# zqqqqz2000/MixGRPO

Hardware: AMD Instinct MI355X
Metric: GRPO train-step images/sec, FLUX.1-dev 1024^2 (higher is better)
Workload: dtype bf16

## Files before the change

### mixgrpo_amd/csrc/gemm.hip

```cpp
#include "../../include/mixgrpo_hip.h"
#include "common.h"

#include <cmath>
#include <cstdlib>

namespace {

constexpr int BM = 128, BN = 128, BK = 64;
constexpr int NT = 256;

struct RowMap {
  long ld;
  long rpb;
  long bstride;
};

__device__ __forceinline__ long row_off(const RowMap& r, long m) {
  const uint32_t rpb = (uint32_t)r.rpb;
  const uint32_t b = (uint32_t)m / rpb;
  return (long)b * r.bstride + (long)((uint32_t)m - b * rpb) * r.ld;
}

enum Epi { EPI_BIAS = 0, EPI_BIAS_GELU = 1, EPI_BIAS_GATE_RES = 2, EPI_F32_ACC = 3, EPI_BIAS_MULAUX = 4,
           EPI_QKNORM = 5 ,
// ... 458 lines not shown
  for (int j = 0; j < AHEAD; ++j) load_cs(j, j, dep0);
  __builtin_amdgcn_sched_barrier(0);
  float ssq[MT];
#pragma unroll
  for (int j = 0; j < MT; ++j) {
    float x[16], p[8];
    unpack8(y[j][0], x);
    unpack8(y[j][1], x + 8);
#pragma unroll
    for (int i = 0; i < 8; ++i)
      p[i] = PAIRED ? vadd1(vmul1(x[2 * i], x[2 * i]), vmul1(x[2 * i + 1], x[2 * i + 1])) : x[2 * i] * x[2 * i] + x[2 * i + 1] * x[2 * i + 1];
    float sacc = PAIRED ? vadd1(vadd1(vadd1(p[0], p[1]), vadd1(p[2], p[3])), vadd1(vadd1(p[4], p[5]), vadd1(p[6], p[7])))
                        : ((p[0] + p[1]) + (p[2] + p[3])) + ((p[4] + p[5]) + (p[6] + p[7]));
    sacc += __shfl_xor(sacc, 16, 64);
    sacc += __shfl_xor(sacc, 32, 64);
    ssq[j] = sacc;
    if (j & 1) __builtin_amdgcn_sched_barrier(0);
  }
  {
    float* wr = reinterpret_cast<float*>(red + (wu ^ 1) * 1024);
    const float* rd = reinterpret_cast<const float*>(red + wu * 1024);
    if (fq == 0) {
#pragma unroll
      for (int j = 0; j < MT; ++j) wr[fr + 16 * j] = ssq[j];
    }
    __builtin_amdgcn_sched_barrier(0);
    asm volatile("s_waitcnt lgkmcnt(0)" ::: "memory");
    __builtin_amdgcn_s_barrier();
    __builtin_amdgcn_sched_barrier(0);
#pragma unroll
    for (int j = 0; j < MT; ++j) ssq[j] = ssq[j] + rd[fr + 16 * j];
  }
  bf16_raw* out = (sec ? g.qn_K : g.qn_Q) + (((long)bu * g.qn_H + head) * g.qn_S + g.qn_s0 + t0 + fr) * 128 + hb;
#pragma unroll
  for (int j = 0; j < MT; ++j) {
    const int slot = j % NSLOT;
    if (j + AHEAD < MT) {
      uint32_t dep = 0;
      if (j > 0) asm volatile("" : "+v"(dep) : "v"(y[j - 1][1].w));
      load_cs((j + AHEAD) % NSLOT, j + AHEAD, dep);
    }
    __builtin_amdgcn_sched_barrier(0);
    const float r = rsqrtf(ssq[j] / 128.f + 1e-6f);
    float x[16], o[16];
    unpack8(y[j][0], x);
    unpack8(y[j][1], x + 8);
    if constexpr (PAIRED) {
#pragma unroll
      for (int q4 = 0; q4 < 4; ++q4) {
        const float4 v = cs[slot][q4];
#pragma unroll
        for (int h = 0; h < 2; ++h) {
          const int i = 2 * q4 + h;
          const float cv = h ? v.z : v.x, sv = h ? v.w : v.y;
          const float y0 = vmul1(vmul1(x[2 * i], r), wv[2 * i]), y1 = vmul1(vmul1(x[2 * i + 1], r), wv[2 * i + 1]);
          o[2 * i] = vsub1(vmul1(y0, cv), vmul1(y1, sv));
          o[2 * i + 1] = vadd1(vmul1(y1, cv), vmul1(y0, sv));
        }
      }
    } else {
#pragma unroll
      for (int q4 = 0; q4 < 4; ++q4) {
        const float4 cv = cs[slot][q4], sv = cs[slot][4 + q4];
        const float c[4] = {cv.x, cv.y, cv.z, cv.w}, sn[4] = {sv.x, sv.y, sv.z, sv.w};
#pragma unroll
        for (int h = 0; h < 2; ++h) {
          const int i = 2 * q4 + h;
          const float y0 = x[2 * i] * r * wv[2 * i], y1 = x[2 * i + 1] * r * wv[2 * i + 1];
          o[2 * i] = y0 * c[2 * h] - y1 * sn[2 * h];
          o[2 * i + 1] = y1 * c[2 * h + 1] + y0 * sn[2 * h + 1];
        }
      }
    }
    y[j][0] = pack8(o);
    y[j][1] = pack8(o + 8);
    if (inside) {
      *reinterpret_cast<uint4*>(out + (long)j * 16 * 128 + f0) = y[j][0];
      *reinterpret_cast<uint4*>(out + (long)j * 16 * 128 + f1) = y[j][1];
    }
    __builtin_amdgcn_sched_barrier(0);
  }
}

template <int EPI>
__device__ __forceinline__ void persist_epilogue(const GemmArgs& g, f32x4 (&acc)[4][8], int wid, int lane, long m0,
                                                 long n0, char* red = nullptr) {
  if constexpr (EPI == EPI_QKNORM || EPI == EPI_QKNORM_P) {
    qknorm_epilogue<EPI == EPI_QKNORM_P>(g, acc, wid, lane, m0, n0, red);
    return;
  }
  constexpr int MT = 8;
  const int wm = wid >> 2, wn = wid & 3, fr = lane & 15, fq = lane >> 4;
  const long nw = n0 + wn * 64;
  const long mrow0 = m0 + wm * 128 + fr;

  if (EPI == EPI_F32_ACC) {
    float* Cb = reinterpret_cast<float*>(g.C);
    const bool rmw = g.beta != 0.f;
    bool nok[4];
    long ncol[4];
#pragma unroll
    for (int t = 0; t < 4; ++t) {
      nok[t] = nw + lane_feat(fq, t) < g.N;
      ncol[t] = nok[t] ? nw + lane_feat(fq, t) : 0;
    }
#pragma unroll
    for (int jb = 0; jb < MT; jb += 2) {
      long off[2];
      bool rok[2];
      float4 old[2][4];
#pragma unroll
      for (int jj = 0; jj < 2; ++jj) {
        const long m = mrow0 + (jb + jj) * 16;
        rok[jj] = m < g.M;
        off[jj] = rok[jj] ? row_off(g.c, m) : 0;
      }
      if (rmw) {
#pragma unroll
        for (int jj = 0; jj < 2; ++jj)
#pragma unroll
          for (int t = 0; t < 4; ++t) old[jj][t] = *reinterpret_cast<const float4*>(Cb + off[jj] + ncol[t]);
      }
#pragma unroll
      for (int jj = 0; jj < 2; ++jj)
#pragma unroll
        for (int t = 0; t < 4; ++t) {
          const f32x4 a = acc[t][jb + jj];
          float4 o = make_float4(a[0], a[1], a[2], a[3]);
          if (rmw) {
            o.x = vfma1(g.beta, old[jj][t].x, o.x);
            o.y = vfma1(g.beta, old[jj][t].y, o.y);
            o.z = vfma1(g.beta, old[jj][t].z, o.z);
            o.w = vfma1(g.beta, old[jj][t].w, o.w);
          }
          if (rok[jj] && nok[t]) *reinterpret_cast<float4*>(Cb + off[jj] + ncol[t]) = o;
        }
    }
    return;
  }

  if (!g.rowwise_ok) {
#pragma unroll
    for (int j = 0; j < MT; ++j) {
      const long m = mrow0 + j * 16;
      if (m >= g.M) continue;
      const long crow = row_off(g.c, m);
      const long bidx = (uint32_t)m / (uint32_t)g.c.rpb;
#pragma unroll
      for (int t = 0; t < 4; ++t) {
        const long nn = nw + lane_feat(fq, t);
        if (nn >= g.N) continue;
        float v[4] = {acc[t][j][0], acc[t][j][1], acc[t][j][2], acc[t][j][3]};
        if (g.bias) {
          const uint2 bb = *reinterpret_cast<const uint2*>(g.bias + nn);
          v[0] += bf2f(bb.x & 0xffff); v[1] += bf2f(bb.x >> 16); v[2] += bf2f(bb.y & 0xffff); v[3] += bf2f(bb.y >> 16);
        }
#pragma unroll
        for (int r = 0; r < 4; ++r) v[r] = rbf(v[r]);
        bf16_raw* cp = reinterpret_cast<bf16_raw*>(g.C) + crow + nn;
        uint2 pre;
        pre.x = (uint32_t)f2bf(v[0]) | ((uint32_t)f2bf(v[1]) << 16);
        pre.y = (uint32_t)f2bf(v[2]) | ((uint32_t)f2bf(v[3]) << 16);
        if (EPI == EPI_BIAS_GELU) {
          if (g.aux) *reinterpret_cast<uint2*>(g.aux + m * g.ldaux + nn) = pre;
#pragma unroll
          for (int r = 0; r < 4; ++r) v[r] = gelu_tanh_f(v[r]);
        } else if (EPI == EPI_BIAS_GATE_RES) {
          if (g.aux) *reinterpret_cast<uint2*>(g.aux + m * g.ldaux + nn) = pre;
          const uint2 gg = *reinterpret_cast<const uint2*>(g.gate + bidx * g.gate_ld + nn);
// ... 63 lines not shown
    }
  };
  if (SIDE) {
    load_side(0, 0, 0);
    load_side(1, 2, 0);
  }
  __builtin_amdgcn_sched_barrier(0);
  uint4 y[MT][2];
  {
    float bias[16];
    unpack8(bias0, bias);
    unpack8(bias1, bias + 8);
    if (brows) {
#pragma unroll
      for (int j = 0; j < MT; ++j) {
        float v[16];
#pragma unroll
        for (int t = 0; t < 4; ++t)
#pragma unroll
          for (int r = 0; r < 4; ++r) v[t * 4 + r] = acc[t][j][r] + brow[j];
        y[j][0] = pack8(v);
        y[j][1] = pack8(v + 8);
        __builtin_amdgcn_sched_barrier(0);
      }
    } else {
#pragma unroll
      for (int j = 0; j < MT; ++j) {
        float v[16];
#pragma unroll
        for (int t = 0; t < 4; ++t)
#pragma unroll
          for (int r = 0; r < 4; ++r) v[t * 4 + r] = acc[t][j][r] + bias[t * 4 + r];
        y[j][0] = pack8(v);
        y[j][1] = pack8(v + 8);
        __builtin_amdgcn_sched_barrier(0);
      }
    }
  }
#pragma unroll
  for (int jb = 0; jb < MT; jb += 2) {
    const int slot = (jb >> 1) & 1;
    uint4 o[2][2];
#pragma unroll
    for (int jj = 0; jj < 2; ++jj) {
      const int j = jb + jj;
      if (EPI == EPI_BIAS) {
        o[jj][0] = y[j][0];
        o[jj][1] = y[j][1];
      } else {
        float v[16];
        unpack8(y[j][0], v);
        unpack8(y[j][1], v + 8);
        if (EPI == EPI_BIAS_GELU) {
#pragma unroll
          for (int e = 0; e < 16; ++e) v[e] = gelu_tanh_f(v[e]);
        } else if (EPI == EPI_BIAS_GATE_RES) {
          float gv[16], rv[16];
          unpack8(gate0, gv);
          unpack8(gate1, gv + 8);
          unpack8(side[slot][SIDE ? jj : 0][0], rv);
          unpack8(side[slot][SIDE ? jj : 0][1], rv + 8);
#pragma unroll
          for (int e = 0; e < 16; ++e) v[e] = rv[e] + rbf(gv[e] * v[e]);
        } else if (EPI == EPI_BIAS_MULAUX) {
          float pv[16];
          unpack8(side[slot][SIDE ? jj : 0][0], pv);
          unpack8(side[slot][SIDE ? jj : 0][1], pv + 8);
#pragma unroll
          for (int e = 0; e < 16; ++e) v[e] *= gelu_tanh_grad_f(pv[e]);
        }
        o[jj][0] = pack8(v);
        o[jj][1] = pack8(v + 8);
      }
    }
    if (SIDE && jb + 4 < MT) {
      uint32_t dep = 0;
      asm volatile("" : "+v"(dep) : "v"(o[1][1].w));
      load_side(slot, jb + 4, dep);
    }
#pragma unroll
    for (int jj = 0; jj < 2; ++jj) {
      const int j = jb + jj;
      const int r = fr + 16 * j;
      if (r <= rmax) {
        char* cb = const_cast<char*>(cbase);
        const uint32_t co = (uint32_t)r * ldc2;
        if ((EPI == EPI_BIAS_GELU || EPI == EPI_BIAS_GATE_RES) && g.aux) {
          char* ab = const_cast<char*>(abase);
          const uint32_t ao = (uint32_t)r * lda2;
          if (nok0) *reinterpret_cast<uint4*>(ab + (ao + c0)) = y[j][0];
          if (nok1) *reinterpret_cast<uint4*>(ab + (ao + c1)) = y[j][1];
        }
        if (nok0) *reinterpret_cast<uint4*>(cb + (co + c0)) = o[jj][0];
        if (nok1) *reinterpret_cast<uint4*>(cb + (co + c1)) = o[jj][1];
      }
    }
    __builtin_amdgcn_sched_barrier(0);
  }
}


constexpr int SK_PMAX = 8;
constexpr long SK_SLOT = 256L * 256;

__host__ __device__ inline int sk_parts(int R, int nw) { return R > 0 ? (nw / R < SK_PMAX ? nw / R : SK_PMAX) : 0; }
__host__ __device__ inline bool sk_on(const float* ws, int minparts, int R, int nw, int nkt) {
  const int P = sk_parts(R, nw);
  return ws != nullptr && P >= 2 && P >= minparts && nkt >= 4 * P;
}

struct SkTail {
  int nfull;
  int nseg;
  int tile0, k00, k01, part0;
  int tile1, k11;
};

__device__ __forceinline__ SkTail sk_tail(const GemmArgs& g, int xcnt, int nw, int w, int nkt) {
  SkTail t;
  t.nfull = xcnt / nw;
  const int R = xcnt - t.nfull * nw, base = t.nfull * nw;
  t.nseg = 0; t.tile0 = 0; t.k00 = 0; t.k01 = nkt; t.part0 = 0; t.tile1 = 0; t.k11 = nkt;
  if (!sk_on(g.sk_ws, g.sk_minparts, R, nw, nkt)) {
    if (w < R) { t.nseg = 1; t.tile0 = base + w; }
    return t;
  }
  const int P = sk_parts(R, nw);
  if (w >= P * R) return t;
  const int p = w / R, r = w - p * R;
  t.nseg = 1; t.tile0 = base + r;
  t.k00 = p * nkt / P; t.k01 = (p + 1) * nkt / P;
  t.part0 = 1;
  return t;
}

template <int EPI, bool PAIR>
__global__ void __launch_bounds__(64) gemm_sk_fixup_kernel(GemmArgs g, int nw) {
  const int lane = threadIdx.x, wid = blockIdx.x & 7, xcd = (blockIdx.x >> 3) & 7, r = blockIdx.x >> 6;
  const int tiles_m = (g.M + 255) / 256, tiles_n = (g.N + 255) / 256, nwg = tiles_m * tiles_n, nkt = g.K / BK;
  const int q = nwg >> 3, rem = nwg & 7;
  const int xbeg = xcd < rem ? xcd * (q + 1) : rem * (q + 1) + (xcd - rem) * q;
  const int xcnt = xcd < rem ? q + 1 : q;
  const int nfull = xcnt / nw, R = xcnt - nfull * nw;
  if (r >= R || !sk_on(g.sk_ws, g.sk_minparts, R, nw, nkt)) return;
  const int P = sk_parts(R, nw);
  f32x4 acc[4][8];
#pragma unroll
  for (int i = 0; i < 4; ++i)
#pragma unroll
    for (int j = 0; j < 8; ++j) acc[i][j] = f32x4{0.f, 0.f, 0.f, 0.f};
  for (int p = 0; p < P; ++p) {
    const int w = p * R + r;
    const float* wsp = g.sk_ws + ((long)(w * 8 + xcd) << 16) + ((wid * 32) * 64 + lane) * 4;
#pragma unroll
    for (int i = 0; i < 4; ++i)
#pragma unroll
      for (int j = 0; j < 8; ++j) {
        const f32x4 v = *reinterpret_cast<const f32x4*>(wsp + (i * 8 + j) * 256);
        acc[i][j] += v;
      }
  }
  const int tl = xbeg + nfull * nw + r, band = g.band;
  const int per_band = band * tiles_n, b0 = tl / per_band, rows_in_band = min(band, tiles_m - b0 * band);
  const int in_band = tl - b0 * per_band;
  long m0 = (long)(b0 * band + in_band % rows_in_band) * 256;
  const long n0 = (long)(in_band / rows_in_band) * 256;
  const GemmArgs gl = seg_args<PAIR>(g, m0);
  if constexpr (EPI != EPI_QKNORM && EPI != EPI_QKNORM_P) persist_epilogue<EPI>(gl, acc, wid, lane, m0, n0);
}

template <int EPI, bool CONV, int MODE>
__global__ void __launch_bounds__(512, 2) gemm_pp_kernel(GemmArgs g) {
  constexpr bool SK = (MODE & 1) != 0, PAIR = (MODE & 2) != 0;
  constexpr int TM = 256, TN = 256, NTHR = 512, RS = NTHR / 8, TB = TM * 128, MT = 8, NTL = 4;
  constexpr int WBASE = 3 * TB;
  extern __shared__ __attribute__((aligned(16))) char smem[];
  const int tid = threadIdx.x, lane = tid & 63, wid = tid >> 6;
  const int wm = wid >> 2, wn = wid & 3;
  const int fr = lane & 15, fq = lane >> 4;
  const int tiles_m = (g.M + TM - 1) / TM, tiles_n = (g.N + TN - 1) / TN;
  const int nwg = tiles_m * tiles_n;
  const int nkt = g.K / BK;
  const int band = g.band;
  const int xcd = blockIdx.x & 7, lane_in_xcd = blockIdx.x >> 3, per_xcd_wg = gridDim.x >> 3;
  const int q = nwg >> 3, rem = nwg & 7;
  const int xbeg = xcd < rem ? xcd * (q + 1) : rem * (q + 1) + (xcd - rem) * q;
  const int xcnt = xcd < rem ? q + 1 : q;
  SkTail sk;
  if (SK) {
    sk = sk_tail(g, xcnt, per_xcd_wg, lane_in_xcd, nkt);
  } else {
    sk.nfull = lane_in_xcd < xcnt ? (xcnt - lane_in_xcd + per_xcd_wg - 1) / per_xcd_wg : 0;
    sk.nseg = 0; sk.tile0 = 0; sk.k00 = 0; sk.k01 = nkt; sk.part0 = 0; sk.tile1 = 0; sk.k11 = nkt;
  }
  const int nunits = sk.nfull + sk.nseg;
  if (nunits == 0) return;
  const int wu = __builtin_amdgcn_readfirstlane(wid);
  const bool late = wu >= 4;
  const int lrow = tid >> 3, lkc = tid & 7;
  const int src_kc = swz(lrow, lkc);
  const int wrow = wperm(lrow);
  typedef __attribute__((address_space(3))) char lds_char;
  typedef const __attribute__((address_space(1))) char gbl_char;
  uint32_t ao[4], wo[4];
  long m0, n0;
#define TILE_COORDS(tl, M0, N0)                                            \
  do {                                                                     \
    const int per_band = band * tiles_n;                                   \
    const int b0 = (tl) / per_band;                                        \
    const int rows_in_band = min(band, tiles_m - b0 * band);               \
    const int in_band = (tl) - b0 * per_band;                              \
    M0 = (long)(b0 * band + in_band % rows_in_band) * TM;                  \
    N0 = (long)(in_band / rows_in_band) * TN;                              \
  } while (0)
#define TILE_OFFS(M0, N0, AO, WO)                                                          \
  do {                                                                                     \
    _Pragma("unroll") for (int k_ = 0; k_ < 4; ++k_) {                                     \
      long mm = M0 + lrow + k_ * RS;                                                       \
      if (mm >= g.M) mm = g.M - 1;                                                         \
      const bool s2_ = PAIR && g.m_split && M0 >= g.m_split;                               \
      const long ar_ = !PAIR ? row_off(g.a, mm)                                            \
                             : (s2_ ? row_off(g.a2, mm - g.m_split) + g.a2_off : row_off(g.a, mm) + g.a1_off); \
      AO[k_] = (uint32_t)((ar_ + src_kc * 8) * 2);                                         \
      long nn = N0 + k_ * 64 + wrow;                                                       \
      if (nn >= g.N) nn = g.N - 1;                                                         \
      WO[k_] = (uint32_t)((nn * g.ldw + (!PAIR ? 0 : (s2_ ? g.w2_off : g.w1_off)) + src_kc * 8) * 2); \
    }                                                                                      \
  } while (0)
#define PGLDS(base, off, off_lds) \
  __builtin_amdgcn_global_load_lds((gbl_char*)((base) + (off)), (lds_char*)(smem + (off_lds)), 16, 0, 0)
#define PIN() __builtin_amdgcn_sched_barrier(0)
#define BAR() do { PIN(); __builtin_amdgcn_s_barrier(); PIN(); } while (0)

  uint32_t a_ro[2], w_ro[2];
#pragma unroll
  for (int ks = 0; ks < 2; ++ks) {
    a_ro[ks] = (uint32_t)((wm * 128 + fr) * 128 + (swz(fr, ks * 4 + fq) << 4));
    w_ro[ks] = (uint32_t)(WBASE + (wn * 64 + fr) * 128 + (swz(fr, ks * 4 + fq) << 4));
  }
#define LDA(ks, j) (*reinterpret_cast<const s16x8*>(smem + sa_ + a_ro[ks] + (j) * 2048))
#define LDW(ks, i) (*reinterpret_cast<const s16x8*>(smem + sw_ + w_ro[ks] + (i) * 2048))
#define MMA(i_, j_, W_, A_) acc[i_][j_] = __builtin_amdgcn_mfma_f32_16x16x32_bf16(W_, A_, acc[i_][j_], 0, 0, 0)

#define PGLDS_K PGLDS
#define LDA_K LDA
#define LDW_K LDW
#define UNIT(i, T_, K0_, K1_, P_)                                                        \
  do {                                                                                     \
    const int s_ = SK ? (i) - sk.nfull : -1;                                               \
    T_ = s_ < 0 ? lane_in_xcd + (i) * per_xcd_wg : (s_ == 0 ? sk.tile0 : sk.tile1);       \
    K0_ = s_ < 0 ? 0 : (s_ == 0 ? sk.k00 : 0);                                             \
    K1_ = s_ < 0 ? nkt : (s_ == 0 ? sk.k01 : sk.k11);                                      \
    P_ = s_ < 0 ? 0 : (s_ == 0 ? sk.part0 : 1);                                            \
  } while (0)
  int ui = 0, u_tile, kbeg, kend, partial;
  UNIT(0, u_tile, kbeg, kend, partial);
  TILE_COORDS(xbeg + u_tile, m0, n0);
  TILE_OFFS(m0, n0, ao, wo);
  {
    const char* ab = reinterpret_cast<const char*>(g.A);
    const char* wb = reinterpret_cast<const char*>(g.W) + (long)kbeg * (BK * 2);
    const int la = wu * 1024, lw = WBASE + wu * 1024;
#pragma unroll
    for (int k = 0; k < 4; ++k) PGLDS(ab + a_koff<CONV>(g, kbeg) * 2, ao[k], la + k * RS * 128);
#pragma unroll
    for (int k = 0; k < 4; ++k) PGLDS(wb, wo[k], lw + k * RS * 128);
#pragma unroll
    for (int k = 0; k < 4; ++k) PGLDS(ab + a_koff<CONV>(g, kbeg + 1) * 2, ao[k], TB + la + k * RS * 128);
#pragma unroll
    for (int k = 0; k < 4; ++k) PGLDS(wb + BK * 2, wo[k], TB + lw + k * RS * 128);
  }
  asm volatile("s_waitcnt vmcnt(0)" ::: "memory");
  __syncthreads();
  if (late) __builtin_amdgcn_s_barrier();
  int aslot = 0, wslot = 0;
  while (true) {
    const bool has_next = ui + 1 < nunits;
    long nm0 = 0, nn0 = 0;
    int n_tile = u_tile, nkbeg = kbeg, nkend = kend, npartial = partial;
    uint32_t nao[4] = {ao[0], ao[1], ao[2], ao[3]}, nwo[4] = {wo[0], wo[1], wo[2], wo[3]};
    if (has_next) {
      UNIT(ui + 1, n_tile, nkbeg, nkend, npartial);
      TILE_COORDS(xbeg + n_tile, nm0, nn0);
      TILE_OFFS(nm0, nn0, nao, nwo);
    }
    uint32_t ca[4] = {ao[0], ao[1], ao[2], ao[3]}, cw[4] = {wo[0], wo[1], wo[2], wo[3]};
    f32x4 acc[NTL][MT];
#pragma unroll
    for (int i = 0; i < NTL; ++i)
#pragma unroll
      for (int j = 0; j < MT; ++j) acc[i][j] = f32x4{0.f, 0.f, 0.f, 0.f};
    const int klen = kend - kbeg;
    for (int kt = 0; kt < klen; ++kt) {
      const bool nxt = kt + 2 >= klen;
      const int k2 = nxt ? nkbeg + (kt + 2 - klen) : kbeg + kt + 2;
#pragma unroll
      for (int k = 0; k < 4; ++k) {
        ca[k] = nxt ? nao[k] : ca[k];
        cw[k] = nxt ? nwo[k] : cw[k];
      }
      const int a_dst = aslot == 0 ? 2 : aslot - 1;
      const char* ab_ = reinterpret_cast<const char*>(g.A) + a_koff<CONV>(g, k2) * 2;
      const char* wb_ = reinterpret_cast<const char*>(g.W) + (long)k2 * (BK * 2);
      const int la_ = a_dst * TB + wu * 1024, lw_ = WBASE + wslot * TB + wu * 1024;
      const uint32_t sa_ = aslot * TB, sw_ = wslot * TB;
      s16x8 faA[2][4], faB[2][4], fw[2][4];
#pragma unroll
      for (int ks = 0; ks < 2; ++ks)
#pragma unroll
        for (int i = 0; i < 4; ++i) fw[ks][i] = LDW_K(ks, i);
#pragma unroll
      for (int ks = 0; ks < 2; ++ks)
#pragma unroll
        for (int j = 0; j < 4; ++j) faA[ks][j] = LDA_K(ks, j);
#pragma unroll
      for (int k = 0; k < 4; ++k) PGLDS_K(ab_, ca[k], la_ + k * RS * 128);
      BAR();
      __builtin_amdgcn_s_setprio(1);
#pragma unroll
      for (int ks = 0; ks < 2; ++ks)
#pragma unroll
        for (int j = 0; j < 4; ++j)
#pragma unroll
          for (int i = 0; i < 4; ++i) MMA(i, j, fw[ks][i], faA[ks][j]);
      __builtin_amdgcn_s_setprio(0);
      BAR();
#pragma unroll
      for (int ks = 0; ks < 2; ++ks)
#pragma unroll
        for (int j = 0; j < 4; ++j) faB[ks][j] = LDA_K(ks, 4 + j);
#pragma unroll
      for (int k = 0; k < 4; ++k) PGLDS_K(wb_, cw[k], lw_ + k * RS * 128);
      PIN();
      asm volatile("s_waitcnt vmcnt(8)" ::: "memory");
      BAR();
      __builtin_amdgcn_s_setprio(1);
#pragma unroll
      for (int ks = 0; ks < 2; ++ks)
#pragma unroll
        for (int j = 0; j < 4; ++j)
#pragma unroll
          for (int i = 0; i < 4; ++i) MMA(i, 4 + j, fw[ks][i], faB[ks][j]);
      __builtin_amdgcn_s_setprio(0);
      BAR();
      aslot = aslot == 2 ? 0 : aslot + 1;
      wslot ^= 1;
    }
    int el = lane, ew = wid;
    asm volatile("" : "+v"(el), "+v"(ew));
    if (SK && partial) {
      float* wsp = g.sk_ws + ((long)blockIdx.x << 16) + ((ew * 32) * 64 + el) * 4;
#pragma unroll
      for (int i = 0; i < NTL; ++i)
#pragma unroll
        for (int j = 0; j < MT; ++j) *reinterpret_cast<f32x4*>(wsp + (i * MT + j) * 256) = acc[i][j];
    } else if (PAIR) {
      long m0l = m0;
      const GemmArgs gl = seg_args<true>(g, m0l);
      persist_epilogue<EPI>(gl, acc, ew, el, m0l, n0);
    } else {
      persist_epilogue<EPI>(g, acc, ew, el, m0, n0, smem + (aslot == 0 ? 2 : aslot - 1) * TB);
    }
    if (!has_next) break;
    ++ui;
    u_tile = n_tile; kbeg = nkbeg; kend = nkend; partial = npartial;
    m0 = nm0; n0 = nn0;
#pragma unroll
    for (int k = 0; k < 4; ++k) { ao[k] = nao[k]; wo[k] = nwo[k]; }
  }
  if (!late) __builtin_amdgcn_s_barrier();
#undef UNIT
#undef TILE_COORDS
#undef TILE_OFFS
#undef PGLDS
#undef PIN
#undef BAR
#undef PGLDS_K
#undef LDA_K
#undef LDW_K
#undef LDA
#undef LDW
#undef MMA
}

bool persistent_ok(const GemmArgs& g) {
  const long tiles_big = (long)cdiv(g.M, 256) * cdiv(g.N, 256);
  static const long min_tiles = getenv("MGX_GEMM_BIG_MIN_TILES") ? atol(getenv("MGX_GEMM_BIG_MIN_TILES")) : 128;
  static const int mode = getenv("MGX_GEMM_MODE") ? atoi(getenv("MGX_GEMM_MODE")) : 9;
  const bool big = g.M >= 256 && g.N >= 256 && tiles_big >= min_tiles && (g.N % 256 == 0 || g.N >= 2048);
  return big && mode != 0 && g.span32 && g.K >= 2 * BK;
}

template <int EPI, bool CONV = false>
int launch(const GemmArgs& g_in, hipStream_t st) {
  GemmArgs g = g_in;
  {
    const int tiles_m = cdiv(g.M, 256), tiles_n = cdiv(g.N, 256);
    static const int band_env = getenv("MGX_GEMM_BAND") ? atoi(getenv("MGX_GEMM_BAND")) : 0;
    g.band = band_env > 0 ? min(band_env, tiles_m) : (g.band > 0 ? min(g.band, tiles_m) : (tiles_n <= 16 ? 1 : (tiles_m <= 16 ? tiles_m : 4)));
  }
  const long tiles_big = (long)cdiv(g.M, 256) * cdiv(g.N, 256);
  static bool attr_set = false;
  if (!attr_set) {
    (void)hipFuncSetAttribute((const void*)gemm_kernel<EPI, CONV>, hipFuncAttributeMaxDynamicSharedMemorySize, 65536);
    (void)hipFuncSetAttribute((const void*)gemm_pp_kernel<EPI, CONV, 0>, hipFuncAttributeMaxDynamicSharedMemorySize, 163840);
    if (!CONV) {
      (void)hipFuncSetAttribute((const void*)gemm_pp_kernel<EPI, false, 1>, hipFuncAttributeMaxDynamicSharedMemorySize, 163840);
      (void)hipFuncSetAttribute((const void*)gemm_pp_kernel<EPI, false, 2>, hipFuncAttributeMaxDynamicSharedMemorySize, 163840);
      (void)hipFuncSetAttribute((const void*)gemm_pp_kernel<EPI, false, 3>, hipFuncAttributeMaxDynamicSharedMemorySize, 163840);
    }
    attr_set = true;
  }
  const bool pair = !CONV && g.m_split != 0;
  if (EPI == EPI_QKNORM || EPI == EPI_QKNORM_P) g.sk_ws = nullptr;
  if (persistent_ok(g)) {
    int grid = 256;
    static const float sk_cost_us = getenv("MGX_GEMM_SK_COST_US") ? (float)atof(getenv("MGX_GEMM_SK_COST_US")) : 40.f;
    static const float sk_slow = getenv("MGX_GEMM_SK_SLOWDOWN") ? (float)atof(getenv("MGX_GEMM_SK_SLOWDOWN")) : 1.25f;
    static const int sk_off = getenv("MGX_GEMM_SK") ? atoi(getenv("MGX_GEMM_SK")) == 0 : 0;
    int rmax = 0;
    g.sk_minparts = 0;
    if (g.sk_ws && !sk_off && !CONV) {
      const float tile_us = (float)g.K * 0.0247f;
      const float room = 1.f - sk_cost_us / tile_us;
      g.sk_minparts = room <= 0.f ? SK_PMAX + 1 : (int)floorf(sk_slow / room) + 1;
      if (g.sk_minparts < 2) g.sk_minparts = 2;
      const int nw = grid / 8, q = (int)(tiles_big >> 3), rem = (int)(tiles_big & 7);
      for (int x = 0; x < 8; ++x) {
        const int cnt = x < rem ? q + 1 : q, R = cnt % nw;
        if (sk_on(g.sk_ws, g.sk_minparts, R, nw, g.K / BK) && R > rmax) rmax = R;
      }
    }
    if (rmax == 0) {
      g.sk_ws = nullptr;
      if (tiles_big < grid) grid = (int)((tiles_big + 7) / 8 * 8);
    }
    if (rmax > 0 && pair) {
      gemm_pp_kernel<EPI, false, 3><<<grid, 512, 163840, st>>>(g);
      gemm_sk_fixup_kernel<EPI, true><<<rmax * 64, 64, 0, st>>>(g, grid / 8);
    } else if (rmax > 0) {
      gemm_pp_kernel<EPI, false, 1><<<grid, 512, 163840, st>>>(g);
      gemm_sk_fixup_kernel<EPI, false><<<rmax * 64, 64, 0, st>>>(g, grid / 8);
    } else if (pair) {
      gemm_pp_kernel<EPI, false, 2><<<grid, 512, 163840, st>>>(g);
    } else {
      gemm_pp_kernel<EPI, CONV, 0><<<grid, 512, 163840, st>>>(g);
    }
  } else {
    if (pair) return 1;
    gemm_kernel<EPI, CONV><<<cdiv(g.M, BM) * cdiv(g.N, BN), NT, 65536, st>>>(g);
  }
  MGX_CHECK_LAUNCH();
  return MGX_OK;
}

__global__ void __launch_bounds__(256) gelu_rows_kernel(const bf16_raw* __restrict__ x, long ldx, bf16_raw* __restrict__ y,
                                                        long ldy, long M, int N8) {
  const long total = M * N8;
  for (long id = (long)blockIdx.x * 256 + threadIdx.x; id < total; id += (long)gridDim.x * 256) {
    const long m = id / N8;
    const int c = (int)(id - m * N8);
    const uint4 u = *reinterpret_cast<const uint4*>(x + m * ldx + c * 8);
    float v[8];
    unpack8(u, v);
#pragma unroll
    for (int e = 0; e < 8; ++e) v[e] = gelu_tanh_f(v[e]);
    *reinterpret_cast<uint4*>(y + m * ldy + c * 8) = pack8(v);
  }
}

}

extern "C" long mgx_gemm_sk_workspace_elems(void) { return 256L * SK_SLOT; }

namespace {
int dispatch(const GemmArgs& g, int epilogue, hipStream_t st) {
  switch (epilogue) {
    case EPI_BIAS: return launch<EPI_BIAS>(g, st);
    case EPI_BIAS_GELU: return launch<EPI_BIAS_GELU>(g, st);
    case EPI_BIAS_GATE_RES: return launch<EPI_BIAS_GATE_RES>(g, st);
    case EPI_F32_ACC: return launch<EPI_F32_ACC>(g, st);
    case EPI_BIAS_MULAUX: return launch<EPI_BIAS_MULAUX>(g, st);
  }
  mgx_set_error("unknown GEMM epilogue");
  return MGX_ERR_ARG;
}

bool side_ok16(int N, int M, const void* C, long ldc, long c_rpb, long c_bstride, const void* aux, long ldaux, const void* gate,
               long gate_ld, const void* bias) {
  return (N % 8 == 0) && (c_rpb >= M || c_rpb % 128 == 0) && (ldc % 8 == 0) && (c_bstride % 8 == 0) && ((uintptr_t)C % 16 == 0) &&
         (!aux || (ldaux % 8 == 0 && (uintptr_t)aux % 16 == 0)) && (!gate || (gate_ld % 8 == 0 && (uintptr_t)gate % 16 == 0)) &&
         (!bias || (uintptr_t)bias % 16 == 0);
}
}

extern "C" int mgx_gemm_bf16_sk(const uint16_t* A, const uint16_t* W, const uint16_t* bias, void* C, const uint16_t* gate,
                                uint16_t* aux, long ldaux, int M, int N, int K, long lda, long a_rpb, long a_bstride, long ldw, long ldc,
                                long c_rpb, long c_bstride, long gate_ld, int epilogue, float beta, float* sk_workspace,
                                long sk_workspace_elems, void* stream) {
  MGX_REQUIRE(A && W && C, "null operand");
  MGX_REQUIRE(!sk_workspace || (sk_workspace_elems >= mgx_gemm_sk_workspace_elems() && (uintptr_t)sk_workspace % 16 == 0),
              "stream-K workspace too small (mgx_gemm_sk_workspace_elems) or misaligned");
  MGX_REQUIRE(M > 0 && N > 0 && K > 0, "empty GEMM");
  MGX_REQUIRE(K % BK == 0, "K must be a multiple of 64");
  MGX_REQUIRE(N % 4 == 0, "N must be a multiple of 4");
  MGX_REQUIRE(lda % 8 == 0 && ldw % 8 == 0 && ldc % 4 == 0, "leading dimensions must keep 16-byte row alignment");
  MGX_REQUIRE(a_rpb > 0 && c_rpb > 0, "rows-per-batch must be positive");
  MGX_REQUIRE(!aux || ldaux % 4 == 0, "aux leading dimension must keep 8-byte alignment");
  MGX_REQUIRE(a_bstride % 8 == 0 && c_bstride % 4 == 0, "batch strides must keep alignment");
  MGX_REQUIRE(((uintptr_t)A % 16 == 0) && ((uintptr_t)W % 16 == 0) && ((uintptr_t)C % 8 == 0), "operands must be 16-byte aligned");
  MGX_REQUIRE(epilogue != EPI_BIAS_GATE_RES || gate, "gate-residual epilogue needs a gate");
  MGX_REQUIRE(epilogue != EPI_BIAS_MULAUX || aux, "gelu-backward epilogue needs the saved pre-activation");
  GemmArgs g{};
  g.A = A; g.W = W; g.bias = bias; g.C = C; g.gate = gate; g.aux = aux; g.ldaux = ldaux; g.gate_ld = gate_ld;
  g.M = M; g.N = N; g.K = K;
  const long RPB_MAX = 1L << 30;
  g.a = RowMap{lda, a_rpb < RPB_MAX ? a_rpb : RPB_MAX, a_bstride};
  g.c = RowMap{ldc, c_rpb < RPB_MAX ? c_rpb : RPB_MAX, c_bstride};
  g.ldw = ldw;
  g.beta = beta;
// ... 201 lines not shown
```

Baseline: 0.4341.

## Defer persistent GEMM epilogue stores into next tile's K-loop

In the persistent GEMM, the bf16 epilogue output of a full interior tile is kept in registers instead of being written right away. The global stores are then issued in batches during the first peeled K-iterations of the next tile, so the store traffic overlaps with MFMA work. The first MMA zeroes the accumulator in place of a separate clear, and the vmcnt waits are adjusted to cover the pending stores. The cost is more register pressure (16 uint4 per lane) and tight hand-tuned waitcnt schedules. It is enabled by default for the BIAS and BIAS_GATE_RES epilogues.

```diff
diff --git a/mixgrpo_amd/csrc/gemm.hip b/mixgrpo_amd/csrc/gemm.hip
--- a/mixgrpo_amd/csrc/gemm.hip
+++ b/mixgrpo_amd/csrc/gemm.hip
@@ -564,9 +564,15 @@
   }
 }
 
-template <int EPI>
+struct PendAddr {
+  char* cb;
+  uint32_t ldc2;
+  uint32_t off0;
+};
+template <int EPI, bool DEFER = false>
 __device__ __forceinline__ void persist_epilogue(const GemmArgs& g, f32x4 (&acc)[4][8], int wid, int lane, long m0,
-                                                 long n0, char* red = nullptr) {
+                                                 long n0, char* red = nullptr, uint4 (*pend)[2] = nullptr,
+                                                 PendAddr* pa = nullptr) {
   if constexpr (EPI == EPI_QKNORM || EPI == EPI_QKNORM_P) {
     qknorm_epilogue<EPI == EPI_QKNORM_P>(g, acc, wid, lane, m0, n0, red);
     return;
@@ -796,20 +802,30 @@
     for (int jj = 0; jj < 2; ++jj) {
       const int j = jb + jj;
       const int r = fr + 16 * j;
-      if (r <= rmax) {
+      if (DEFER || r <= rmax) {
         char* cb = const_cast<char*>(cbase);
         const uint32_t co = (uint32_t)r * ldc2;
         if ((EPI == EPI_BIAS_GELU || EPI == EPI_BIAS_GATE_RES) && g.aux) {
           char* ab = const_cast<char*>(abase);
           const uint32_t ao = (uint32_t)r * lda2;
-          if (nok0) *reinterpret_cast<uint4*>(ab + (ao + c0)) = y[j][0];
-          if (nok1) *reinterpret_cast<uint4*>(ab + (ao + c1)) = y[j][1];
+          if (DEFER || nok0) *reinterpret_cast<uint4*>(ab + (ao + c0)) = y[j][0];
+          if (DEFER || nok1) *reinterpret_cast<uint4*>(ab + (ao + c1)) = y[j][1];
         }
-        if (nok0) *reinterpret_cast<uint4*>(cb + (co + c0)) = o[jj][0];
-        if (nok1) *reinterpret_cast<uint4*>(cb + (co + c1)) = o[jj][1];
+        if constexpr (DEFER) {
+          pend[j][0] = o[jj][0];
+          pend[j][1] = o[jj][1];
+        } else {
+          if (nok0) *reinterpret_cast<uint4*>(cb + (co + c0)) = o[jj][0];
+          if (nok1) *reinterpret_cast<uint4*>(cb + (co + c1)) = o[jj][1];
+        }
       }
     }
     __builtin_amdgcn_sched_barrier(0);
+  }
+  if constexpr (DEFER) {
+    pa->cb = const_cast<char*>(cbase);
+    pa->ldc2 = (uint32_t)__builtin_amdgcn_readfirstlane((int)ldc2);
+    pa->off0 = (uint32_t)fr * ldc2 + c0;
   }
 }
 
@@ -883,9 +899,32 @@
   if constexpr (EPI != EPI_QKNORM && EPI != EPI_QKNORM_P) persist_epilogue<EPI>(gl, acc, wid, lane, m0, n0);
 }
 
-template <int EPI, bool CONV, int MODE>
+constexpr int defer_s(int epi, int i) {
+#ifdef MGX_DEFER_SCHED
+  constexpr int s[4] = MGX_DEFER_SCHED;
+  return s[i];
+#else
+  constexpr int wide[4] = {2, 1, 1, 0}, tight[4] = {2, 2, 0, 0};
+  return epi == EPI_BIAS_GATE_RES ? wide[i] : tight[i];
+#endif
+}
+constexpr int DEFER_BST = 4;
+constexpr int DEFER_AUX = 16;
+constexpr int DEFER_MINK = 4;
+constexpr bool defer_epi(int epi) { return epi == EPI_BIAS || epi == EPI_BIAS_GELU || epi == EPI_BIAS_GATE_RES || epi == EPI_BIAS_MULAUX; }
+
+template <int EPI, bool CONV, int MODE, bool DEFER = false>
 __global__ void __launch_bounds__(512, 2) gemm_pp_kernel(GemmArgs g) {
   constexpr bool SK = (MODE & 1) != 0, PAIR = (MODE & 2) != 0;
+  static_assert(!DEFER || (defer_epi(EPI) && !CONV), "only the four bf16 epilogues of the plain GEMM defer their stores");
+  constexpr int DEFER_S[4] = {defer_s(EPI, 0), defer_s(EPI, 1), defer_s(EPI, 2), defer_s(EPI, 3)};
+  constexpr int DEFER_W0 = 8 + DEFER_BST * (DEFER_S[0] + DEFER_S[1]);
+  constexpr int DEFER_W1 = 8 + DEFER_BST * (DEFER_S[1] + DEFER_S[2] + DEFER_S[3]);
+  constexpr int DEFER_W2 = 8 + DEFER_BST * DEFER_S[3];
+  constexpr int DEFER_PEEL = DEFER_S[3] > 0 ? 3 : 2;
+  static_assert(DEFER_S[0] + DEFER_S[1] + DEFER_S[2] + DEFER_S[3] == 4, "a wave's block is four 2-row batches");
+  static_assert(DEFER_W0 + DEFER_AUX <= 63 && DEFER_W1 <= 63 && DEFER_W2 <= 63, "vmcnt is a 6-bit counter");
+  static_assert(DEFER_PEEL + 1 <= DEFER_MINK, "the peeled K-iterations must exist");
   constexpr int TM = 256, TN = 256, NTHR = 512, RS = NTHR / 8, TB = TM * 128, MT = 8, NTL = 4;
   constexpr int WBASE = 3 * TB;
   extern __shared__ __attribute__((aligned(16))) char smem[];
@@ -954,7 +993,27 @@
   }
 #define LDA(ks, j) (*reinterpret_cast<const s16x8*>(smem + sa_ + a_ro[ks] + (j) * 2048))
 #define LDW(ks, i) (*reinterpret_cast<const s16x8*>(smem + sw_ + w_ro[ks] + (i) * 2048))
-#define MMA(i_, j_, W_, A_) acc[i_][j_] = __builtin_amdgcn_mfma_f32_16x16x32_bf16(W_, A_, acc[i_][j_], 0, 0, 0)
+#define MMA(i_, j_, W_, A_, Z_) \
+  acc[i_][j_] = __builtin_amdgcn_mfma_f32_16x16x32_bf16(W_, A_, (Z_) ? f32x4{0.f, 0.f, 0.f, 0.f} : acc[i_][j_], 0, 0, 0)
+  constexpr bool EPI_HAS_AUX = EPI == EPI_BIAS_GELU || EPI == EPI_BIAS_GATE_RES;
+  uint4 pend[8][2];
+  PendAddr pa;
+  bool carry = false, p_aux = false;
+#define PEND_CLEAR()                                                                                    \
+  do {                                                                                                  \
+    _Pragma("unroll") for (int j_ = 0; j_ < 8; ++j_) pend[j_][0] = pend[j_][1] = make_uint4(0, 0, 0, 0); \
+  } while (0)
+  PEND_CLEAR();
+  pa.cb = nullptr; pa.ldc2 = 0; pa.off0 = 0;
+#define PEND_STORE(b_)                                                                                  \
+  do {                                                                                                  \
+    _Pragma("unroll") for (int jj_ = 0; jj_ < 2; ++jj_) {                                               \
+      const int j_ = 2 * (b_) + jj_;                                                                    \
+      const uint32_t co_ = pa.off0 + (uint32_t)(16 * j_) * pa.ldc2;                                     \
+      *reinterpret_cast<uint4*>(pa.cb + co_) = pend[j_][0];                                             \
+      *reinterpret_cast<uint4*>(pa.cb + (co_ + 64)) = pend[j_][1];                                      \
+    }                                                                                                   \
+  } while (0)
 
 #define PGLDS_K PGLDS
 #define LDA_K LDA
@@ -1000,68 +1059,96 @@
     }
     uint32_t ca[4] = {ao[0], ao[1], ao[2], ao[3]}, cw[4] = {wo[0], wo[1], wo[2], wo[3]};
     f32x4 acc[NTL][MT];
-#pragma unroll
-    for (int i = 0; i < NTL; ++i)
-#pragma unroll
-      for (int j = 0; j < MT; ++j) acc[i][j] = f32x4{0.f, 0.f, 0.f, 0.f};
     const int klen = kend - kbeg;
-    for (int kt = 0; kt < klen; ++kt) {
-      const bool nxt = kt + 2 >= klen;
-      const int k2 = nxt ? nkbeg + (kt + 2 - klen) : kbeg + kt + 2;
-#pragma unroll
-      for (int k = 0; k < 4; ++k) {
-        ca[k] = nxt ? nao[k] : ca[k];
-        cw[k] = nxt ? nwo[k] : cw[k];
-      }
-      const int a_dst = aslot == 0 ? 2 : aslot - 1;
-      const char* ab_ = reinterpret_cast<const char*>(g.A) + a_koff<CONV>(g, k2) * 2;
-      const char* wb_ = reinterpret_cast<const char*>(g.W) + (long)k2 * (BK * 2);
-      const int la_ = a_dst * TB + wu * 1024, lw_ = WBASE + wslot * TB + wu * 1024;
-      const uint32_t sa_ = aslot * TB, sw_ = wslot * TB;
-      s16x8 faA[2][4], faB[2][4], fw[2][4];
-#pragma unroll
-      for (int ks = 0; ks < 2; ++ks)
-#pragma unroll
-        for (int i = 0; i < 4; ++i) fw[ks][i] = LDW_K(ks, i);
-#pragma unroll
-      for (int ks = 0; ks < 2; ++ks)
-#pragma unroll
-        for (int j = 0; j < 4; ++j) faA[ks][j] = LDA_K(ks, j);
-#pragma unroll
-      for (int k = 0; k < 4; ++k) PGLDS_K(ab_, ca[k], la_ + k * RS * 128);
-      BAR();
-      __builtin_amdgcn_s_setprio(1);
-#pragma unroll
-      for (int ks = 0; ks < 2; ++ks)
-#pragma unroll
-        for (int j = 0; j < 4; ++j)
-#pragma unroll
-          for (int i = 0; i < 4; ++i) MMA(i, j, fw[ks][i], faA[ks][j]);
-      __builtin_amdgcn_s_setprio(0);
-      BAR();
-#pragma unroll
-      for (int ks = 0; ks < 2; ++ks)
-#pragma unroll
-        for (int j = 0; j < 4; ++j) faB[ks][j] = LDA_K(ks, 4 + j);
-#pragma unroll
-      for (int k = 0; k < 4; ++k) PGLDS_K(wb_, cw[k], lw_ + k * RS * 128);
-      PIN();
-      asm volatile("s_waitcnt vmcnt(8)" ::: "memory");
-      BAR();
-      __builtin_amdgcn_s_setprio(1);
-#pragma unroll
-      for (int ks = 0; ks < 2; ++ks)
-#pragma unroll
-        for (int j = 0; j < 4; ++j)
-#pragma unroll
-          for (int i = 0; i < 4; ++i) MMA(i, 4 + j, fw[ks][i], faB[ks][j]);
-      __builtin_amdgcn_s_setprio(0);
-      BAR();
-      aslot = aslot == 2 ? 0 : aslot + 1;
-      wslot ^= 1;
-    }
+#define KITER(Z_, B0_, NA_, NB_, WAIT_)                                                                     \
+    {                                                                                                       \
+      const bool nxt = kt + 2 >= klen;                                                                      \
+      const int k2 = nxt ? nkbeg + (kt + 2 - klen) : kbeg + kt + 2;                                         \
+      _Pragma("unroll") for (int k = 0; k < 4; ++k) {                                                       \
+        ca[k] = nxt ? nao[k] : ca[k];                                                                       \
+        cw[k] = nxt ? nwo[k] : cw[k];                                                                       \
+      }                                                                                                     \
+      const int a_dst = aslot == 0 ? 2 : aslot - 1;                                                         \
+      const char* ab_ = reinterpret_cast<const char*>(g.A) + a_koff<CONV>(g, k2) * 2;                       \
+      const char* wb_ = reinterpret_cast<const char*>(g.W) + (long)k2 * (BK * 2);                           \
+      if (DEFER) {                 \
+        asm volatile("" : "+s"(ab_));                                                                       \
+        asm volatile("" : "+s"(wb_));                                                                       \
+      }                                                                                                     \
+      const int la_ = a_dst * TB + wu * 1024, lw_ = WBASE + wslot * TB + wu * 1024;                         \
+      const uint32_t sa_ = aslot * TB, sw_ = wslot * TB;                                                    \
+      s16x8 faA[2][4], faB[2][4], fw[2][4];                                                                 \
+                                                                                               \
+      _Pragma("unroll") for (int ks = 0; ks < 2; ++ks)                                                      \
+        _Pragma("unroll") for (int i = 0; i < 4; ++i) fw[ks][i] = LDW_K(ks, i);                             \
+      _Pragma("unroll") for (int ks = 0; ks < 2; ++ks)                                                      \
+        _Pragma("unroll") for (int j = 0; j < 4; ++j) faA[ks][j] = LDA_K(ks, j);                            \
+      _Pragma("unroll") for (int k = 0; k < 4; ++k) PGLDS_K(ab_, ca[k], la_ + k * RS * 128);                \
+      if (NA_ > 0) {                                                                                        \
+        PIN();                                                                                              \
+        _Pragma("unroll") for (int b_ = 0; b_ < NA_; ++b_) PEND_STORE(B0_ + b_);                            \
+      }                                                                                                     \
+      BAR();                                                                                                \
+                                                                  \
+      __builtin_amdgcn_s_setprio(1);                                                                        \
+      _Pragma("unroll") for (int ks = 0; ks < 2; ++ks)                                                      \
+        _Pragma("unroll") for (int j = 0; j < 4; ++j)                                                       \
+          _Pragma("unroll") for (int i = 0; i < 4; ++i) MMA(i, j, fw[ks][i], faA[ks][j], Z_ && ks == 0);    \
+      __builtin_amdgcn_s_setprio(0);                                                                        \
+      BAR();                                                                                                \
+                                                                                               \
+      _Pragma("unroll") for (int ks = 0; ks < 2; ++ks)                                                      \
+        _Pragma("unroll") for (int j = 0; j < 4; ++j) faB[ks][j] = LDA_K(ks, 4 + j);                        \
+      _Pragma("unroll") for (int k = 0; k < 4; ++k) PGLDS_K(wb_, cw[k], lw_ + k * RS * 128);                \
+      if (NB_ > 0) {                                                                                        \
+        PIN();                                                                                              \
+        _Pragma("unroll") for (int b_ = 0; b_ < NB_; ++b_) PEND_STORE(B0_ + NA_ + b_);                      \
+      }                                                                                                     \
+      PIN();                                                                                                \
+      WAIT_;                                                                                                \
+      BAR();                                                                                                \
+                                                                \
+      __builtin_amdgcn_s_setprio(1);                                                                        \
+      _Pragma("unroll") for (int ks = 0; ks < 2; ++ks)                                                      \
+        _Pragma("unroll") for (int j = 0; j < 4; ++j)                                                       \
+          _Pragma("unroll") for (int i = 0; i < 4; ++i) MMA(i, 4 + j, fw[ks][i], faB[ks][j], Z_ && ks == 0); \
+      __builtin_amdgcn_s_setprio(0);                                                                        \
+      BAR();                                                                                                \
+      aslot = aslot == 2 ? 0 : aslot + 1;                                                                   \
+      wslot ^= 1;                                                                                           \
+    }
+#define VMWAIT(N_)                                                                                          \
+    do {                                                                                                    \
+      if (DEFER) __builtin_amdgcn_s_waitcnt(((N_) & 15) | (((N_) >> 4) << 14) | (7 << 4) | (15 << 8));      \
+      else asm volatile("s_waitcnt vmcnt(%0)" ::"n"(N_) : "memory");                                        \
+    } while (0)
+    int kt = 0;
+    if (DEFER && carry) {
+      KITER(true, 0, DEFER_S[0], DEFER_S[1],
+            if (EPI_HAS_AUX && p_aux) VMWAIT(DEFER_W0 + DEFER_AUX); else VMWAIT(DEFER_W0));
+      kt = 1;
+      KITER(false, DEFER_S[0] + DEFER_S[1], DEFER_S[2], DEFER_S[3], VMWAIT(DEFER_W1));
+      kt = 2;
+      if constexpr (DEFER_PEEL == 3) {
+        KITER(false, 4, 0, 0, VMWAIT(DEFER_W2));
+        kt = 3;
+      }
+    } else {
+#pragma unroll
+      for (int i = 0; i < NTL; ++i)
+#pragma unroll
+        for (int j = 0; j < MT; ++j) acc[i][j] = f32x4{0.f, 0.f, 0.f, 0.f};
+    }
+    for (; kt < klen; ++kt) KITER(false, 0, 0, 0, VMWAIT(8));
+#undef KITER
     int el = lane, ew = wid;
     asm volatile("" : "+v"(el), "+v"(ew));
+    const bool defer_next = DEFER && g.rowwise_ok && has_next && !(SK && (partial || npartial)) && nkend - nkbeg >= DEFER_MINK;
+    if constexpr (DEFER) {
+      carry = false;
+      PEND_CLEAR();
+      pa.cb = nullptr; pa.ldc2 = 0; pa.off0 = 0;
+    }
     if (SK && partial) {
       float* wsp = g.sk_ws + ((long)blockIdx.x << 16) + ((ew * 32) * 64 + el) * 4;
 #pragma unroll
@@ -1071,7 +1158,21 @@
     } else if (PAIR) {
       long m0l = m0;
       const GemmArgs gl = seg_args<true>(g, m0l);
-      persist_epilogue<EPI>(gl, acc, ew, el, m0l, n0);
+      if constexpr (DEFER) {
+        carry = defer_next && m0l + (wu >> 2) * 128 + 128 <= gl.M && n0 + (wu & 3) * 64 + 64 <= gl.N;
+        p_aux = gl.aux != nullptr;
+        if (carry) persist_epilogue<EPI, true>(gl, acc, ew, el, m0l, n0, nullptr, pend, &pa);
+        else persist_epilogue<EPI>(gl, acc, ew, el, m0l, n0);
+      } else {
+        persist_epilogue<EPI>(gl, acc, ew, el, m0l, n0);
+      }
+    } else if (DEFER) {
+      if constexpr (DEFER) {
+        carry = defer_next && m0 + (wu >> 2) * 128 + 128 <= g.M && n0 + (wu & 3) * 64 + 64 <= g.N;
+        p_aux = g.aux != nullptr;
+        if (carry) persist_epilogue<EPI, true>(g, acc, ew, el, m0, n0, nullptr, pend, &pa);
+        else persist_epilogue<EPI>(g, acc, ew, el, m0, n0);
+      }
     } else {
       persist_epilogue<EPI>(g, acc, ew, el, m0, n0, smem + (aslot == 0 ? 2 : aslot - 1) * TB);
     }
@@ -1095,6 +1196,9 @@
 #undef LDA
 #undef LDW
 #undef MMA
+#undef PEND_STORE
+#undef PEND_CLEAR
+#undef VMWAIT
 }
 
 bool persistent_ok(const GemmArgs& g) {
@@ -1114,6 +1218,9 @@
     g.band = band_env > 0 ? min(band_env, tiles_m) : (g.band > 0 ? min(g.band, tiles_m) : (tiles_n <= 16 ? 1 : (tiles_m <= 16 ? tiles_m : 4)));
   }
   const long tiles_big = (long)cdiv(g.M, 256) * cdiv(g.N, 256);
+  constexpr bool DEFER_OK = !CONV && defer_epi(EPI);
+  static const int defer_mode = getenv("MGX_GEMM_DEFER_EPI") ? atoi(getenv("MGX_GEMM_DEFER_EPI")) : 1;
+  static const bool defer_on = DEFER_OK && (defer_mode >= 2 || (defer_mode == 1 && (EPI == EPI_BIAS || EPI == EPI_BIAS_GATE_RES)));
   static bool attr_set = false;
   if (!attr_set) {
     (void)hipFuncSetAttribute((const void*)gemm_kernel<EPI, CONV>, hipFuncAttributeMaxDynamicSharedMemorySize, 65536);
@@ -1122,6 +1229,12 @@
       (void)hipFuncSetAttribute((const void*)gemm_pp_kernel<EPI, false, 1>, hipFuncAttributeMaxDynamicSharedMemorySize, 163840);
       (void)hipFuncSetAttribute((const void*)gemm_pp_kernel<EPI, false, 2>, hipFuncAttributeMaxDynamicSharedMemorySize, 163840);
       (void)hipFuncSetAttribute((const void*)gemm_pp_kernel<EPI, false, 3>, hipFuncAttributeMaxDynamicSharedMemorySize, 163840);
+    }
+    if constexpr (DEFER_OK) {
+      (void)hipFuncSetAttribute((const void*)gemm_pp_kernel<EPI, false, 0, true>, hipFuncAttributeMaxDynamicSharedMemorySize, 163840);
+      (void)hipFuncSetAttribute((const void*)gemm_pp_kernel<EPI, false, 1, true>, hipFuncAttributeMaxDynamicSharedMemorySize, 163840);
+      (void)hipFuncSetAttribute((const void*)gemm_pp_kernel<EPI, false, 2, true>, hipFuncAttributeMaxDynamicSharedMemorySize, 163840);
+      (void)hipFuncSetAttribute((const void*)gemm_pp_kernel<EPI, false, 3, true>, hipFuncAttributeMaxDynamicSharedMemorySize, 163840);
     }
     attr_set = true;
   }
@@ -1149,7 +1262,21 @@
       g.sk_ws = nullptr;
       if (tiles_big < grid) grid = (int)((tiles_big + 7) / 8 * 8);
     }
-    if (rmax > 0 && pair) {
+    const bool defer = defer_on && g.rowwise_ok && tiles_big > grid;
+    if constexpr (DEFER_OK) {
+      if (defer) {
+        if (rmax > 0 && pair) gemm_pp_kernel<EPI, false, 3, true><<<grid, 512, 163840, st>>>(g);
+        else if (rmax > 0) gemm_pp_kernel<EPI, false, 1, true><<<grid, 512, 163840, st>>>(g);
+        else if (pair) gemm_pp_kernel<EPI, false, 2, true><<<grid, 512, 163840, st>>>(g);
+        else gemm_pp_kernel<EPI, false, 0, true><<<grid, 512, 163840, st>>>(g);
+      }
+    }
+    if (defer) {
+      if (rmax > 0) {
+        if (pair) gemm_sk_fixup_kernel<EPI, true><<<rmax * 64, 64, 0, st>>>(g, grid / 8);
+        else gemm_sk_fixup_kernel<EPI, false><<<rmax * 64, 64, 0, st>>>(g, grid / 8);
+      }
+    } else if (rmax > 0 && pair) {
       gemm_pp_kernel<EPI, false, 3><<<grid, 512, 163840, st>>>(g);
       gemm_sk_fixup_kernel<EPI, true><<<rmax * 64, 64, 0, st>>>(g, grid / 8);
     } else if (rmax > 0) {
```

Result: no change. 0.4370 (median of 6 runs) (+0.7%).
